# heng-hw/SpaCap3D

Hardware: AMD Instinct MI355X
Metric: scenes/sec (40k pts, 256 proposals) fwd+bwd (higher is better)
Workload: dtype f32; 1 GPU; cfg2: synthetic ScanRefer-shaped scans, 40000 pts x (xyz+1 ch), 256 proposals, 8 scenes/GPU; full training step (SpaCapNet fwd + loss + bwd + grad all-reduce + Adam); global_batch=8, parallelism=dp1, hip_graph=True, fps_prefetch_side_stream=True, prefetch_as_graph=True, reserved_cus_forward=8, geometry_prefetch=True, deferred_weight_gradients=True, params=9290918, allreduce_bytes=35572416

## Files before the change

### include/spacap_hip.h

```cpp
#ifndef SPACAP_HIP_H
#define SPACAP_HIP_H

#include <stddef.h>
#include <stdint.h>

#ifdef __cplusplus
extern "C" {
#endif

#define SPACAP_ABI_VERSION 5

#define SPACAP_OK 0
#define SPACAP_E_INVALID (-1)
#define SPACAP_E_LAUNCH (-2)
#define SPACAP_E_NO_DEVICE (-3)

typedef void *spacap_stream_t;

int spacap_abi_version(void);
const char *spacap_last_error(void);
int spacap_device_count(void);

int spacap_opt_n_threads(int work_size);

// ... 199 lines not shown
int spacap_sa_dgrad_l1in_f32(const float *dy, const float *zk, const float *coef, const float *Wk, const float *rel4,
                             const float *W1, int ldw, int has_feat, const float *st_p, int B, int N, int S, double *part,
                             float *part_l1, spacap_stream_t stream);
int spacap_sa_dgrad_wgrad_l1in_slabs(long R);
int spacap_sa_dgrad_wgrad_l1in_f32(const float *dy, const float *zk, const float *coef, const float *Wk, const float *rel4,
                                   const float *W1, int ldw, int has_feat, const float *st_p, int B, int N, int S, double *part,
                                   float *part_l1, float *partW, spacap_stream_t stream);
int spacap_sa_wgrad_f32(const float *dy, const uint8_t *arg, int S, const float *zk, const float *coef,
                        const float *zp, const float *st_p, long R, int CK, int CP, float *partW,
                        spacap_stream_t stream);
int spacap_sa_l1_bwd_f32(float *dy1, const float *z1, const float *coef, const float *feat, const float *xyz,
                         const float *new_xyz, const int32_t *idx, const float *W1, int ldw, float rdiv, int B,
                         int Np, int N, int S, int C1, float *partW, float *drel, int write_dz,
                         spacap_stream_t stream);
size_t spacap_sa_rows_scatter_workspace_bytes(int B, int Np, long E);
int spacap_sa_rows_scatter_f32(const float *dz, const int32_t *idx, int B, int Np, long E, int C, float *out,
                               void *workspace, spacap_stream_t stream);
int spacap_sa_rows_index_f32(const int32_t *idx, int B, int Np, long E, void *workspace, spacap_stream_t stream);
int spacap_sa_rows_gather_f32(const float *dz, int B, int Np, long E, int C, const void *workspace, float *out,
                              spacap_stream_t stream);
int spacap_sa_drel_sums_f32(const float *drel, int B, int Np, int N, int S, const void *workspace, float *dxyz, float *dnew,
                            spacap_stream_t stream);
int spacap_sa_dw1_assemble_f32(const float *pw1, int n1, const float *pf, int nf, int C1, int Cf, float *dW1, spacap_stream_t stream);

int spacap_linear_wgrad_slabs(long R, int CK, int CP);
int spacap_linear_wgrad_f32(const float *g, const float *x, long R, int CK, int CP, int with_bias, float *part,
                            spacap_stream_t stream);
int spacap_linear_wgrad_nslab_f32(const float *g, const float *x, long R, int CK, int CP, int with_bias, int nslab, float *part,
                                  spacap_stream_t stream);
int spacap_linear_wgrad_slabs_batched(long R, int CK, int CP);
int spacap_linear_wgrad_batched_f32(const float *const *g, const float *const *x, const long *R, const int *CK,
                                    const int *CP, const int *with_bias, const int *nslabs, float *const *part, int njobs,
                                    spacap_stream_t stream);

int spacap_relu_dropout_fwd_f32(const float *x, long n, float p, uint64_t seed, const uint64_t *seed_dev,
                                float *out, spacap_stream_t stream);
int spacap_relu_dropout_bwd_f32(const float *g, const float *y, long n, float p, float *dx, spacap_stream_t stream);
int spacap_dropout_add_fwd_f32(const float *res, const float *y, long n, float p, uint64_t seed,
                               const uint64_t *seed_dev, float *out, spacap_stream_t stream);
int spacap_dropout_add_bwd_f32(const float *g, long n, float p, uint64_t seed, const uint64_t *seed_dev,
                               float *out, spacap_stream_t stream);

int spacap_scene_aug_doubles(void);
int spacap_scene_sample_augment_f32(const float *const *scene_feat, const int32_t *const *scene_ins,
                                    const uint8_t *const *scene_isobj, const float *const *scene_color,
                                    const int32_t *choices, const double *aug, int B, int P, int C, int augment,
// ... 295 lines not shown
```

### spacap3d_amd/_native.py

```python
import ctypes
import os

import torch

_HERE = os.path.dirname(os.path.abspath(__file__))
LIB_PATH = os.path.join(_HERE, "lib", "libspacap_hip.so")
ABI_VERSION = 5

_i = ctypes.c_int
_l = ctypes.c_long
_f = ctypes.c_float
_p = ctypes.c_void_p
_u64 = ctypes.c_uint64

SIGNATURES = {
    "spacap_abi_version": (_i, []),
    "spacap_last_error": (ctypes.c_char_p, []),
    "spacap_device_count": (_i, []),
    "spacap_opt_n_threads": (_i, [_i]),
    "spacap_fps_workspace_bytes": (ctypes.c_size_t, [_i, _i]),
    "spacap_fps_f32": (_i, [_p, _i, _i, _i, _p, _p, _p]),
    "spacap_gather_points_f32": (_i, [_p, _p, _i, _i, _i, _i, _p, _p]),
    "spacap_gather_points_grad_f32": (_i, [_p, _p, _i, _i, _i, _i, _p, _p]),
    "spacap_ball_query_f32": (_i, [_p, _p, _i, _i, _i, _f, _i, _p, _p]),
# ... 112 lines not shown
    "spacap_rel_wide_tail_supported": (_i, [_i]),
    "spacap_rel_wide_tail_nparts": (_i, [_l]),
    "spacap_rel_wide_tail_bwd_f32": (_i, [_p, _p, _p, _l, _i, _i, _p, _p, _p]),
    "spacap_rel_wide_l1_supported": (_i, [_i, _i, _i]),
    "spacap_rel_wide_transpose_f32": (_i, [_p, _p, _i, _i, _i, _i, _p]),
    "spacap_rel_wide_l1_fwd_f32": (_i, [_p, _p, _p, _i, _i, _i, _i, _p, _p]),
    "spacap_rel_wide_l1_bwd_f32": (_i, [_p, _p, _p, _p, _i, _i, _i, _i, _p, _p, _p, _p]),
    "spacap_sa_l3bwd_part_floats": (_l, [_i, _i]),
    "spacap_sa_l3bwd_dw_f32": (_i, [_p, _i, _p, _p, _i, _i, _p, _p, _p]),
    "spacap_sa_wgrad_pool_supported": (_i, [_i, _i, _i]),
    "spacap_sa_wgrad_pool_parts": (_i, [_l, _i, _i, _i]),
    "spacap_sa_wgrad_pool_f32": (_i, [_p, _p, _i, _p, _p, _p, _l, _i, _i, _p, _p]),
    "spacap_sa_bwd_finalize_f32": (_i, [_p, _i, _l, _p, _p, _p, _p, _p]),
    "spacap_sa_dgrad_f32": (_i, [_p, _p, _i, _p, _p, _p, _p, _p, _l, _i, _i, _p, _p, _p]),
    "spacap_sa_dgrad_l1_f32": (_i, [_p] * 10 + [_f] + [_i] * 6 + [_p, _p, _p]),
    "spacap_sa_wgrad_f32": (_i, [_p, _p, _i, _p, _p, _p, _p, _l, _i, _i, _p, _p]),
    "spacap_sa_l1_bwd_f32": (_i, [_p, _p, _p, _p, _p, _p, _p, _p, _i, _f, _i, _i, _i, _i, _i, _p, _p, _i, _p]),
    "spacap_sa_rows_scatter_workspace_bytes": (ctypes.c_size_t, [_i, _i, _l]),
    "spacap_sa_rows_scatter_f32": (_i, [_p, _p, _i, _i, _l, _i, _p, _p, _p]),
    "spacap_sa_rows_index_f32": (_i, [_p, _i, _i, _l, _p, _p]),
    "spacap_sa_rows_gather_f32": (_i, [_p, _i, _i, _l, _i, _p, _p, _p]),
    "spacap_sa_drel_sums_f32": (_i, [_p, _i, _i, _i, _i, _p, _p, _p, _p]),
    "spacap_sa_dw1_assemble_f32": (_i, [_p, _i, _p, _i, _i, _i, _p, _p]),
    "spacap_relu_dropout_fwd_f32": (_i, [_p, _l, _f, _u64, _p, _p, _p]),
    "spacap_relu_dropout_bwd_f32": (_i, [_p, _p, _l, _f, _p, _p]),
    "spacap_dropout_add_fwd_f32": (_i, [_p, _p, _l, _f, _u64, _p, _p, _p]),
    "spacap_dropout_add_bwd_f32": (_i, [_p, _l, _f, _u64, _p, _p, _p]),
    "spacap_scene_aug_doubles": (_i, []),
    "spacap_scene_sample_augment_f32": (_i, [_p, _p, _p, _p, _p, _p, _i, _i, _i, _i, _p, _p, _p, _p, _p]),
    "spacap_scene_sample_augment_map_f32": (_i, [_p, _p, _p, _p, _p, _p, _i, _i, _i, _i, _i, _p, _p, _p, _p, _p, _p]),
    "spacap_scene_gather_rows_f32": (_i, [_p, _p, _i, _i, _i, _p, _i, _i, _p]),
    "spacap_l2norm_rows_fwd_f32": (_i, [_p, _l, _i, _p, _p, _p]),
    "spacap_l2norm_rows_bwd_f32": (_i, [_p, _p, _p, _l, _i, _p, _p]),
    "spacap_cap_loss_fwd_f32": (_i, [_p, _p, _p, _i, _i, _i, _i, _p, _p, _p, _p]),
    "spacap_cap_loss_bwd_f32": (_i, [_p, _p, _p, _p, _p, _i, _i, _i, _i, _p, _p]),
    "spacap_scene_votes_workspace_bytes": (ctypes.c_size_t, [_i, _i]),
    "spacap_scene_votes_f32": (_i, [_p, _p, _p, _i, _i, _i, _i, _p, _p, _p, _p]),
    "spacap_det_npart": (_i, []),
    "spacap_det_losses_fwd_f32": (_i, [_p] * 16 + [_i] * 8 + [_f] * 4 + [_p] * 9 + [_p]),
    "spacap_det_losses_bwd_f32": (_i, [_p] * 5 + [_i] * 6 + [_p] * 3 + [_p]),
    "spacap_rel_loss_nparts": (_l, [_i, _i]),
    "spacap_rel_loss_fwd_f32": (_i, [_p] * 7 + [_i] * 3 + [_p] * 3 + [_p]),
    "spacap_rel_loss_bwd_f32": (_i, [_p] * 3 + [_i] * 2 + [_p, _p]),
    "spacap_sum_slabs_f32": (_i, [_p, _i, _l, _p, _p]),
    "spacap_sum_slabs_batched_f32": (_i, [_p, _p, _p, _p, _i, _p]),
    "spacap_adam_flat_f32": (_i, [_p, _p, _p, _p, _l, _f, _f, _f, _f, _f, _p, _f, _p, _p]),
# ... 61 lines not shown
            "`python -c 'import __graft_entry__ as g; g.build()'` (or `make -C spacap3d_amd/csrc`). "
            "spacap3d_amd has no CPU or PyTorch fallback for its native operators.")
    lib = ctypes.CDLL(LIB_PATH)
    for name, (res, args) in SIGNATURES.items():
        fn = getattr(lib, name)
        fn.restype = res
        fn.argtypes = args
    got = lib.spacap_abi_version()
    if got != ABI_VERSION:
        raise ImportError(f"libspacap_hip.so ABI {got} != expected {ABI_VERSION}: rebuild the extension")
    return lib


lib = _load()


def check(rc: int, what: str) -> None:
    if rc != 0:
        msg = lib.spacap_last_error().decode("utf-8", "replace")
        raise RuntimeError(f"{what} failed (code {rc}): {msg}")


_DEFERRED = None


class deferred_slab_sums:

    def __enter__(self):
        global _DEFERRED
        self._prev = _DEFERRED
        self.items = []
        self.jobs = []
        self.conv_jobs = []
        _DEFERRED = self
        return self

    def __exit__(self, *exc):
        global _DEFERRED
        _DEFERRED = self._prev
        if exc[0] is None:
            self.flush()
        return False

    def has_job_for(self, part):
        ptr = part.data_ptr()
        return any(j[3].data_ptr() == ptr for j in self.jobs) or any(j[3].data_ptr() == ptr for j in self.conv_jobs)

    def outputs(self):
        return [o for _, o in self.items]

    def flush(self):
        self.run_jobs()
        self.run_sums()

    def run_jobs(self):
        import torch
        jobs, self.jobs = self.jobs, []
        if jobs:
            by_dev = {}
            for j in jobs:
                by_dev.setdefault(j[0].device, []).append(j)
            for dev, group in by_dev.items():
                k = len(group)
                arr = lambda ct, vals: (ct * k)(*vals)
                with torch.cuda.device(dev):
                    check(lib.spacap_linear_wgrad_batched_f32(
                        arr(ctypes.c_void_p, [j[0].data_ptr() for j in group]), arr(ctypes.c_void_p, [j[1].data_ptr() for j in group]),
                        arr(ctypes.c_long, [j[0].shape[0] for j in group]), arr(ctypes.c_int, [j[0].shape[1] for j in group]),
                        arr(ctypes.c_int, [j[1].shape[1] for j in group]), arr(ctypes.c_int, [int(j[2]) for j in group]),
                        arr(ctypes.c_int, [j[3].shape[0] for j in group]),
                        arr(ctypes.c_void_p, [j[3].data_ptr() for j in group]), k, torch.cuda.current_stream(dev).cuda_stream),
                        "spacap_linear_wgrad_batched_f32")
        cjobs, self.conv_jobs = self.conv_jobs, []
        if cjobs:
            by_dev = {}
            for j in cjobs:
# ... 61 lines not shown
            return out.view(part.shape[1:])
        return part[0]
    can_defer = deferrable and _DEFERRED is not None and part.is_cuda and part.data_ptr() % 16 == 0 and n % 4 == 0 \
        and part.dtype == torch.float32 and part.is_contiguous()
    if not can_defer and _DEFERRED is not None and part.is_cuda and _DEFERRED.has_job_for(part):
        _DEFERRED.run_jobs()
    if not part.is_cuda or n % 4 or part.dtype != torch.float32 or not part.is_contiguous():
        return part.sum(0)
    if can_defer:
        if out is None:
            with torch.cuda.device(part.device):
                out = torch.empty(part.shape[1:], dtype=torch.float32, device=part.device)
        else:
            out = out.view(part.shape[1:])
        _DEFERRED.items.append((part, out))
        return out
    with torch.cuda.device(part.device):
        out = torch.empty(part.shape[1:], dtype=torch.float32, device=part.device) if out is None else out.view(part.shape[1:])
        check(lib.spacap_sum_slabs_f32(part.data_ptr(), part.shape[0], n, out.data_ptr(),
                                       torch.cuda.current_stream(part.device).cuda_stream), "spacap_sum_slabs_f32")
    return out


def linear_wgrad_partials(g2, x2, with_bias, deferrable=False):
    import torch
    R, CK = g2.shape
    CP = x2.shape[1]
    nslab = int(lib.spacap_linear_wgrad_slabs(R, CK, CP))
    if nslab == 0:
        return None
    with torch.cuda.device(g2.device):
        if deferrable and _DEFERRED is not None:
            nb = int(lib.spacap_linear_wgrad_slabs_batched(R, CK, CP))
            part = torch.empty(nb, CK * CP + (CK if with_bias else 0), dtype=torch.float32, device=g2.device)
            _DEFERRED.jobs.append((g2, x2, bool(with_bias), part))
            return part
        part = torch.empty(nslab, CK * CP + (CK if with_bias else 0), dtype=torch.float32, device=g2.device)
        check(lib.spacap_linear_wgrad_f32(g2.data_ptr(), x2.data_ptr(), R, CK, CP, 1 if with_bias else 0, part.data_ptr(),
                                          torch.cuda.current_stream(g2.device).cuda_stream), "spacap_linear_wgrad_f32")
    return part


def conv1x1_wgrad_partials(g, x, B, CO, CI, N, deferrable=False, with_bias=False):
    import torch
    with torch.cuda.device(g.device):
        if deferrable and _DEFERRED is not None:
            nb = int(lib.spacap_conv1x1_wgrad_slabs_batched(B, CO, CI, N))
            part = torch.empty(nb, CO * CI + (((CO + 3) // 4) * 4 if with_bias else 0), dtype=torch.float32, device=g.device)
            _DEFERRED.conv_jobs.append((g, x, (B, CO, CI, N), part, bool(with_bias)))
            return part
        nslab = int(lib.spacap_conv1x1_wgrad_slabs(B, CO, CI, N))
        part = torch.empty(nslab, CO * CI, dtype=torch.float32, device=g.device)
        check(lib.spacap_conv1x1_wgrad_f32(g.data_ptr(), x.data_ptr(), B, CO, CI, N, part.data_ptr(),
                                           torch.cuda.current_stream(g.device).cuda_stream), "spacap_conv1x1_wgrad_f32")
    return part

# ... 20 lines not shown
```

### spacap3d_amd/csrc/sa_bwd.hip

```cpp
#include "sa_common.hpp"

namespace {

__global__ __launch_bounds__(1024) void sa_bwd_finalize_kernel(const double *__restrict__ part, int nparts, int C,
                                                              double M, const float *__restrict__ stats,
                                                              float *__restrict__ coef, float *__restrict__ dgamma,
                                                              float *__restrict__ dbeta) {
  __shared__ double s[64][16];
  const int tid = threadIdx.x, col = tid & 15, slab = tid >> 4;
  const int k = col >> 3, c = blockIdx.x * 8 + (col & 7);
  double a = 0.0;
  if (c < C) {
#pragma unroll 16
    for (int p = slab; p < nparts; p += 64) a += part[((size_t)p * 2 + k) * C + c];
  }
  s[slab][col] = a;
  __syncthreads();
  if (tid < 8 && c < C) {
    double s1 = 0.0, s2 = 0.0;
    for (int i = 0; i < 64; ++i) s1 += s[i][tid], s2 += s[i][tid + 8];
    const float mean = stats[c * 4], istd = stats[c * 4 + 1], g = stats[c * 4 + 2];
    const float a1 = (float)(s1 / M), b1 = (float)(s2 / M);
    const float k1 = g * b1 * istd;
    coef[c * 4 + 0] = g;
// ... 467 lines not shown
        py = dz[0] * wy[0] + dz[1] * wy[1] + dz[2] * wy[2] + dz[3] * wy[3];
        pz = dz[0] * wz[0] + dz[1] * wz[1] + dz[2] * wz[2] + dz[3] * wz[3];
      }
    }
    if (drel) {
#pragma unroll
      for (int o = 1; o < C4; o <<= 1) px += __shfl_xor(px, o), py += __shfl_xor(py, o), pz += __shfl_xor(pz, o);
      if (c4 == 0 && r < R) drel[r * 3] = px / rdiv, drel[r * 3 + 1] = py / rdiv, drel[r * 3 + 2] = pz / rdiv;
    }
  }
  st4(&s_red[0][rs][c4 * 4], ax);
  st4(&s_red[1][rs][c4 * 4], ay);
  st4(&s_red[2][rs][c4 * 4], az);
  st4(&s_red[3][rs][c4 * 4], af);
  __syncthreads();
  for (int e = tid; e < 4 * C1; e += 256) {
    const int c = e / 4, k = e % 4;
    float a = 0.f;
    for (int i = 0; i < RP; ++i) a += s_red[k][i][c];
    partW[((size_t)blockIdx.x * C1 + c) * 4 + k] = a;
  }
}

__global__ __launch_bounds__(256) void sa_dw1_assemble_kernel(const float *__restrict__ pw1, int n1, const float *__restrict__ pf, int nf,
                                                              int C1, int Cf, float *__restrict__ out) {
  __shared__ float s_g[4][64];
  const int c = threadIdx.x & 63, grp = threadIdx.x >> 6;
  const long e = (long)blockIdx.x * 64 + c, ne = (long)C1 * (3 + Cf);
  float a = 0.f;
  if (e < ne) {
    const int ch = (int)(e / (3 + Cf)), j = (int)(e % (3 + Cf));
    const float *src = j < 3 ? pw1 + (size_t)ch * 4 + j : pf + (size_t)ch * Cf + (j - 3);
    const size_t stride = j < 3 ? (size_t)C1 * 4 : (size_t)C1 * Cf;
    const int ns = j < 3 ? n1 : nf, per = (ns + 3) / 4, s0 = grp * per, s1 = min(ns, s0 + per);
    int k = s0;
    for (; k + 32 <= s1; k += 32) {
      float t[32];
#pragma unroll
      for (int u = 0; u < 32; ++u) t[u] = src[(size_t)(k + u) * stride];
#pragma unroll
      for (int u = 0; u < 32; ++u) a += t[u];
    }
#pragma unroll 8
    for (; k < s1; ++k) a += src[(size_t)k * stride];
  }
  s_g[grp][c] = a;
  __syncthreads();
  if (grp == 0 && e < ne) out[e] = (s_g[0][c] + s_g[1][c]) + (s_g[2][c] + s_g[3][c]);
}

}

namespace {
int wgrad_resident(int CK, int CP, bool pooled) {
#define WR(CKB, CPV, PV)                                                        \
  {                                                                             \
    static const int res = resident_blocks(sa_wgrad_kernel<CKB, CPV, PV>, 0);   \
    return res;                                                                 \
  }
  if (pooled && CK % 128 == 0 && CP == 64) WR(128, 64, true)
  if (pooled && CK % 128 == 0 && CP == 128) WR(128, 128, true)
  if (!pooled && CK == 64 && CP == 64) WR(64, 64, false)
  if (!pooled && CK == 128 && CP == 128) WR(128, 128, false)
#undef WR
  return 512;
}
}
extern "C" int spacap_sa_wgrad_slabs(long R, int CK, int CP, int pooled) {
  const int gy = CK >= 128 ? CK / 128 : 1;
  long n = bwd_resident(wgrad_resident(CK, CP, pooled != 0)) / gy, cap = (16L << 20) / ((long)CK * CP), tiles = (R + TW - 1) / TW;
  if (n > cap) n = cap;
// ... 161 lines not shown
  const char *what = "spacap_sa_dgrad_l1in_f32";
  SPACAP_REQUIRE(dy && zk && coef && Wk && rel4 && W1 && st_p && part && part_l1 && ldw >= (has_feat ? 4 : 3), "%s: bad arguments", what);
  const long R = (long)B * N * S;
  L1Args L{nullptr, nullptr, nullptr, nullptr, 1.f, 1, N, S, part_l1, rel4, L1In{W1, ldw, has_feat}, nullptr};
  launch_dgrad_l1<false>(dy, zk, coef, Wk, nullptr, st_p, R, part, L, spacap::as_stream(stream));
  SPACAP_CHECK_LAUNCH(what);
  return SPACAP_OK;
}

extern "C" int spacap_sa_dgrad_wgrad_l1in_slabs(long R) { return R >= 1 ? dgrad_l1_grid<true>(R) : 0; }
extern "C" int spacap_sa_dgrad_wgrad_l1in_f32(const float *dy, const float *zk, const float *coef, const float *Wk, const float *rel4,
                                              const float *W1, int ldw, int has_feat, const float *st_p, int B, int N, int S,
                                              double *part, float *part_l1, float *partW, spacap_stream_t stream) {
  const char *what = "spacap_sa_dgrad_wgrad_l1in_f32";
  SPACAP_REQUIRE(dy && zk && coef && Wk && rel4 && W1 && st_p && part && part_l1 && partW && ldw >= (has_feat ? 4 : 3), "%s: bad arguments", what);
  const long R = (long)B * N * S;
  L1Args L{nullptr, nullptr, nullptr, nullptr, 1.f, 1, N, S, part_l1, rel4, L1In{W1, ldw, has_feat}, partW};
  launch_dgrad_l1<true>(dy, zk, coef, Wk, nullptr, st_p, R, part, L, spacap::as_stream(stream));
  SPACAP_CHECK_LAUNCH(what);
  return SPACAP_OK;
}

namespace {
__global__ __launch_bounds__(256) void sa_l1_dw_kernel(const float *__restrict__ part_l1, int nparts, const float *__restrict__ coef,
                                                       int C1, int ldw, float *__restrict__ dW1) {
  __shared__ double s_lane[12][17];
  __shared__ double s_sum[12];
  const int c = blockIdx.x, tid = threadIdx.x, sidx = tid >> 4, l = tid & 15;
  const int n = C1 * 8 + 4;
  if (sidx < 12) {
    const int e = sidx < 8 ? c * 8 + sidx : C1 * 8 + (sidx - 8);
    double a0 = 0.0, a1 = 0.0, a2 = 0.0, a3 = 0.0;
    int p = l;
    for (; p + 48 < nparts; p += 64) {
      a0 += (double)part_l1[(size_t)p * n + e];
      a1 += (double)part_l1[(size_t)(p + 16) * n + e];
      a2 += (double)part_l1[(size_t)(p + 32) * n + e];
      a3 += (double)part_l1[(size_t)(p + 48) * n + e];
    }
    for (; p < nparts; p += 16) a0 += (double)part_l1[(size_t)p * n + e];
    s_lane[sidx][l] = (a0 + a1) + (a2 + a3);
  }
  __syncthreads();
  if (tid < 12) {
    double a = 0.0;
    for (int i = 0; i < 16; ++i) a += s_lane[tid][i];
    s_sum[tid] = a;
  }
  __syncthreads();
  if (tid < ldw) {
    const double g = coef[c * 4 + 0], k0 = coef[c * 4 + 1], k1 = coef[c * 4 + 2];
    dW1[c * ldw + tid] = (float)(g * s_sum[tid] + k0 * s_sum[8 + tid] - k1 * s_sum[4 + tid]);
  }
}
}
extern "C" int spacap_sa_l1_dw_f32(const float *part_l1, int nparts, const float *coef, int C1, int ldw, float *dW1,
                                   spacap_stream_t stream) {
  const char *what = "spacap_sa_l1_dw_f32";
  SPACAP_REQUIRE(part_l1 && coef && dW1 && nparts >= 1 && C1 >= 1 && C1 <= 512 && ldw >= 1 && ldw <= 4, "%s: bad arguments", what);
  hipLaunchKernelGGL(sa_l1_dw_kernel, dim3(C1), dim3(256), 0, spacap::as_stream(stream), part_l1, nparts, coef, C1, ldw, dW1);
  SPACAP_CHECK_LAUNCH(what);
  return SPACAP_OK;
}

extern "C" int spacap_sa_wgrad_f32(const float *dy, const uint8_t *arg, int S, const float *zk, const float *coef,
                                   const float *zp, const float *st_p, long R, int CK, int CP, float *partW,
                                   spacap_stream_t stream) {
  const char *what = "spacap_sa_wgrad_f32";
  SPACAP_REQUIRE(dy && zk && coef && zp && st_p && partW && R >= 1, "%s: bad arguments", what);
  SPACAP_REQUIRE(!arg || (S >= 1 && R % S == 0), "%s: bad S", what);
  hipStream_t s = spacap::as_stream(stream);
  const int nslab = spacap_sa_wgrad_slabs(R, CK, CP, arg ? 1 : 0);
#define WG(CKB, CPV, PV) \
  hipLaunchKernelGGL((sa_wgrad_kernel<CKB, CPV, PV>), dim3(nslab, CK / CKB), dim3(256), 0, s, dy, arg, S, zk, coef, CK, zp, st_p, R, partW)
  if (arg && CK % 128 == 0 && CP == 64) WG(128, 64, true);
  else if (arg && CK % 128 == 0 && CP == 128) WG(128, 128, true);
  else if (!arg && CK == 64 && CP == 64) WG(64, 64, false);
  else if (!arg && CK == 128 && CP == 128) WG(128, 128, false);
  else SPACAP_REQUIRE(false, "%s: (CK=%d, CP=%d, pooled=%d) unsupported", what, CK, CP, arg ? 1 : 0);
#undef WG
  SPACAP_CHECK_LAUNCH(what);
  return SPACAP_OK;
}
// ... 28 lines not shown
```

### spacap3d_amd/csrc/sa_l3bwd.inc

```

__global__ __launch_bounds__(256) void sa_l3_sum_kernel(const float *__restrict__ partW, int nparts, long n, double *__restrict__ sums) {
  __shared__ double s_l[16][65];
  const int q = threadIdx.x & 15, l = threadIdx.x >> 4;
  const long e0 = (long)blockIdx.x * 64 + q * 4;
  double a[4] = {0.0, 0.0, 0.0, 0.0};
  if (e0 < n) {
    const float *pp = partW + e0;
    int p = l;
    for (; p + 7 * 16 < nparts; p += 8 * 16) {
      f32x4 t[8];
#pragma unroll
      for (int u = 0; u < 8; ++u) t[u] = ld4(pp + (size_t)(p + 16 * u) * n);
#pragma unroll
      for (int u = 0; u < 8; ++u)
#pragma unroll
        for (int k = 0; k < 4; ++k) a[k] += (double)t[u][k];
    }
    for (; p < nparts; p += 16) {
      const f32x4 t = ld4(pp + (size_t)p * n);
#pragma unroll
      for (int k = 0; k < 4; ++k) a[k] += (double)t[k];
    }
  }
#pragma unroll
  for (int k = 0; k < 4; ++k) s_l[l][q * 4 + k] = a[k];
  __syncthreads();
  if (threadIdx.x < 64 && (long)blockIdx.x * 64 + threadIdx.x < n) {
    double v = 0.0;
    for (int i = 0; i < 16; ++i) v += s_l[i][threadIdx.x];
    sums[(long)blockIdx.x * 64 + threadIdx.x] = v;
  }
}

__global__ __launch_bounds__(1024) void sa_l3_dw_kernel(const double *__restrict__ sums, const float *__restrict__ coef3,
                                                        const float *__restrict__ W3, int C3, int C2, float *__restrict__ dW3) {
  __shared__ double s_p[1024];
  const int c = blockIdx.x, k = threadIdx.x % C2, sl = threadIdx.x / C2, nsl = 1024 / C2;
  const double *gram = sums + (size_t)C3 * C2, *cs = gram + (size_t)C2 * C2;
  double acc = 0.0;
  for (int j0 = sl * 8; j0 < C2; j0 += nsl * 8) {
    double gv[8];
    float wv[8];
#pragma unroll
    for (int u = 0; u < 8; ++u) {
      const int j = j0 + u < C2 ? j0 + u : C2 - 1;
      gv[u] = gram[(size_t)j * C2 + k];
      wv[u] = W3[(size_t)c * C2 + j];
    }
#pragma unroll
    for (int u = 0; u < 8; ++u)
      if (j0 + u < C2) acc += (double)wv[u] * gv[u];
  }
  s_p[threadIdx.x] = acc;
  __syncthreads();
  if (threadIdx.x < C2) {
    double v = 0.0;
    for (int i = 0; i < nsl; ++i) v += s_p[i * C2 + threadIdx.x];
    const double k0 = coef3[c * 4 + 1], k1 = coef3[c * 4 + 2];
    dW3[(size_t)c * C2 + threadIdx.x] = (float)(sums[(size_t)c * C2 + threadIdx.x] + k0 * cs[threadIdx.x] - k1 * v);
  }
}

struct WPArgs {
  const float *dym;
  const uint8_t *arg;
  const float *coef3;
  const float *z2;
  const float *st2;
  long R;
  float *partW;
};

template <int W, int C2, int C3, int TMT, int S>
__device__ __forceinline__ void wp_tile(const float *sa, const float *sv, const int *sr, f32x4 (&accG)[C2 / 32 + 1],
                                        float (&sacc)[C3 / (C2 / 16)][C2 / 64], int lane) {
  constexpr int NCL = C2 / 16, CH = C2 / 64, CPL = C2 / 64, NI = C3 / NCL, ND = NCL / 2 + 1, NDW = W < NCL / 2 ? ND : ND - 1;
  constexpr int LDA = C2 + 20, KS = TMT / 4, NG = TMT / S, IPK = NG * NI / KS;
  static_assert((NG * NI) % KS == 0 && NI % 4 == 0 && (IPK % 4 == 0 || 4 % IPK == 0), "sparse items per k step");
  using i32x4 = int __attribute__((ext_vector_type(4)));
  const int l15 = lane & 15, lg = lane >> 4;
  const float *pb = sa + lg * LDA + 4 * l15;
  const float *psp = sa + CPL * lane;
  const f32x4 *qv = reinterpret_cast<const f32x4 *>(sv) + W * (NI / 4);
// ... 167 lines not shown
```

### spacap3d_amd/engine.py

```python
import os

import torch

from . import synthetic as S
from .detector import geometry_pyramid, sampling_pyramid
from .distributed import FlatGradBucket, broadcast_parameters, used_parameters
from .loss_helper import get_scene_cap_loss, start_detection_losses


_STREAMS = {}


def _role_stream(device, role):
    device = torch.device(device)
    key = (device.type, device.index if device.index is not None else torch.cuda.current_device())
    if key not in _STREAMS:
        dev = torch.device("cuda", key[1])
        _STREAMS[key] = {r: torch.cuda.Stream(device=dev) for r in ("side", "capture", "comm", "wgrad", "relation")}
    return _STREAMS[key][role]


class Trainer:
    def __init__(self, model: torch.nn.Module, mean_size_arr, lr: float = 1e-3, weight_decay: float = 1e-5,
                 use_relation: bool = True, split_optimizer: bool = False,
# ... 106 lines not shown
        kw = dict(num_heading_bin=S.NUM_HEADING_BIN, num_size_cluster=S.NUM_SIZE_CLUSTER, mean_size_arr=self.mean_size_arr)
        need = ("vote_label", "center_label")
        early = (lambda d: start_detection_losses(d, **kw)) if all(k in data_dict for k in need) else None
        d = self.model(dict(data_dict), after_proposal=early)
        det_vec = d.get("_det_vec")
        d = get_scene_cap_loss(d, use_relation=self.use_relation, **kw)
        if self._overlap_armed or self._flush_mid:
            marks = [t for t in (det_vec, d.get("aggregated_vote_features"), d.get("aggregated_vote_xyz"))
                     if torch.is_tensor(t) and t.requires_grad]
            for t in marks:
                t.register_hook(self._boundary_hook if self._overlap_armed else self._mid_flush_hook)
        return d

    def _mid_flush_hook(self, grad):
        if self._flush_mid and not self._mid_done:
            self._mid_done = 1
            from . import _native
            dq = _native._DEFERRED
            if dq is not None and grad.is_cuda:
                dev = grad.device
                ws = _role_stream(dev, "wgrad")
                cur = torch.cuda.current_stream(dev)
                ws.wait_stream(cur)
                for j in dq.jobs + dq.conv_jobs:
                    for t in (j[0], j[1], j[3]):
                        t.record_stream(ws)
                for part, out in dq.items:
                    part.record_stream(ws)
                    out.record_stream(ws)
                with torch.cuda.stream(ws):
                    dq.flush()
                self._mid_stream = ws
        return None

    def _setup(self, data_dict):
        bufs = [(b, b.detach().clone()) for b in self.model.buffers()]
        d = self.loss(data_dict)
        used = used_parameters(self.model, d["loss"])
        with torch.no_grad():
            for b, saved in bufs:
                b.copy_(saved)
        used = self._group_qkv(used)
        self._adopt_bn_counters()
        self.bucket = FlatGradBucket(used, views=False)
        kw = dict(lr=self.lr, weight_decay=self.weight_decay, eps=self.adam_eps)
        if used[0].is_cuda:
            from .optim import FlatAdam
            self.optimizer = FlatAdam(self.bucket, **kw)
            self._attach_packed_qkv()
            self._register_grad_slots()
        else:
            self.optimizer = torch.optim.Adam(used, **kw)
# ... 504 lines not shown
```

### spacap3d_amd/sa_mlp.py

```python
import torch
from torch.autograd import Function

from .layout import ChannelMajorOf, point_major_of
from ._native import check, lib, sum_slabs


RECOMPUTE_Z1 = True
L1_MOMENTS = True
POOL_WGRAD = True
POOL_WGRAD_MIN_ROWS = 131072
FUSE_L2_WGRAD = True


def _ptr(t):
    return t.data_ptr() if t is not None else None


_SELFTESTED = set()


def _selftest(dev):
    key = (dev.type, dev.index)
    if key in _SELFTESTED:
        return
    _SELFTESTED.add(key)
    with torch.cuda.device(dev), torch.no_grad():
# ... 147 lines not shown
        nparts = int(lib.spacap_sa_nparts())
        with torch.cuda.device(dev):
            part = torch.empty(nparts * 2 * max(C1, C2, C3), dtype=torch.float64, device=dev)
            coef = [torch.empty(c, 4, **f32) for c in (C1, C2, C3)]
            dg = [torch.empty(c, **f32) for c in (C1, C2, C3)]
            db = [torch.empty(c, **f32) for c in (C1, C2, C3)]

            def finalize(k, C, stats):
                check(lib.spacap_sa_bwd_finalize_f32(part.data_ptr(), C, R, stats.data_ptr(), coef[k].data_ptr(),
                                                     dg[k].data_ptr(), db[k].data_ptr(), st), "spacap_sa_bwd_finalize_f32")

            dym = torch.empty(G, C3, **f32)
            check(lib.spacap_sa_pool_bwd_f32(dout.data_ptr(), out.data_ptr(), arg.data_ptr(), z3.data_ptr(), _ptr(zmax), st3.data_ptr(), G, S, C3,
                                             dym.data_ptr(), part.data_ptr(), st), "spacap_sa_pool_bwd_f32")
            finalize(2, C3, st3)
            dy2 = torch.empty(R, C2, **f32)
            if POOL_WGRAD and R >= POOL_WGRAD_MIN_ROWS and lib.spacap_sa_wgrad_pool_supported(C2, C3, S):
                npw, nfl = int(lib.spacap_sa_wgrad_pool_parts(R, C2, C3, S)), int(lib.spacap_sa_l3bwd_part_floats(C2, C3))
                pw = torch.empty(npw, nfl, **f32)
                check(lib.spacap_sa_wgrad_pool_f32(dym.data_ptr(), arg.data_ptr(), S, coef[2].data_ptr(), z2.data_ptr(),
                                                   st2.data_ptr(), R, C3, C2, pw.data_ptr(), st), "spacap_sa_wgrad_pool_f32")
                sums = torch.empty(nfl, dtype=torch.float64, device=dev)
                dW3 = torch.empty(C3, C2, **f32)
                check(lib.spacap_sa_l3bwd_dw_f32(pw.data_ptr(), npw, coef[2].data_ptr(), W3.data_ptr(), C3, C2, sums.data_ptr(),
                                                 dW3.data_ptr(), st), "spacap_sa_l3bwd_dw_f32")
            else:
                pw = torch.empty(int(lib.spacap_sa_wgrad_slabs(R, C3, C2, 1)), C3, C2, **f32)
                check(lib.spacap_sa_wgrad_f32(dym.data_ptr(), arg.data_ptr(), S, z3.data_ptr(), coef[2].data_ptr(),
                                              z2.data_ptr(), st2.data_ptr(), R, C3, C2, pw.data_ptr(), st), "spacap_sa_wgrad_f32")
                dW3 = sum_slabs(pw, deferrable=True)
            check(lib.spacap_sa_dgrad_f32(dym.data_ptr(), arg.data_ptr(), S, z3.data_ptr(), coef[2].data_ptr(),
                                          W3.data_ptr(), z2.data_ptr(), st2.data_ptr(), R, C3, C2, dy2.data_ptr(),
                                          part.data_ptr(), st), "spacap_sa_dgrad_f32")
            finalize(1, C2, st2)
            has_feat = int(feat is not None)
            fuse_l1 = (not ctx.has_Y) and (not ctx.need_xyz) and C1 == 64 and C2 == 64
            fuse_w2 = fuse_l1 and ctx.recompute and FUSE_L2_WGRAD
            if fuse_w2:
                pw = torch.empty(int(lib.spacap_sa_dgrad_wgrad_l1in_slabs(R)), C2, C1, **f32)
            else:
                pw = torch.empty(int(lib.spacap_sa_wgrad_slabs(R, C2, C1, 0)), C2, C1, **f32)
                if ctx.recompute:
                    check(lib.spacap_sa_wgrad_l1in_f32(dy2.data_ptr(), z2.data_ptr(), coef[1].data_ptr(), z1.data_ptr(), W1.data_ptr(),
                                                       W1.shape[1], has_feat, st1.data_ptr(), R, pw.data_ptr(), st),
                          "spacap_sa_wgrad_l1in_f32")
                else:
                    check(lib.spacap_sa_wgrad_f32(dy2.data_ptr(), None, 0, z2.data_ptr(), coef[1].data_ptr(), z1.data_ptr(),
                                                  st1.data_ptr(), R, C2, C1, pw.data_ptr(), st), "spacap_sa_wgrad_f32")
                dW2 = sum_slabs(pw, deferrable=True)
            if fuse_l1:
                pl1 = torch.empty(nparts, C1 * 8 + 4, **f32)
                if fuse_w2:
                    check(lib.spacap_sa_dgrad_wgrad_l1in_f32(dy2.data_ptr(), z2.data_ptr(), coef[1].data_ptr(), W2.data_ptr(),
                                                             z1.data_ptr(), W1.data_ptr(), W1.shape[1], has_feat, st1.data_ptr(), B, N, S,
                                                             part.data_ptr(), pl1.data_ptr(), pw.data_ptr(), st),
                          "spacap_sa_dgrad_wgrad_l1in_f32")
                    dW2 = sum_slabs(pw, deferrable=True)
                elif ctx.recompute:
                    check(lib.spacap_sa_dgrad_l1in_f32(dy2.data_ptr(), z2.data_ptr(), coef[1].data_ptr(), W2.data_ptr(),
                                                       z1.data_ptr(), W1.data_ptr(), W1.shape[1], has_feat, st1.data_ptr(), B, N, S,
                                                       part.data_ptr(), pl1.data_ptr(), st), "spacap_sa_dgrad_l1in_f32")
                else:
                    check(lib.spacap_sa_dgrad_l1_f32(dy2.data_ptr(), z2.data_ptr(), coef[1].data_ptr(), W2.data_ptr(),
                                                     z1.data_ptr(), st1.data_ptr(), _ptr(feat), xyz.data_ptr(),
                                                     new_xyz.data_ptr(), idx.data_ptr(), ctx.rdiv, B, Np, N, S, C2, C1,
                                                     part.data_ptr(), pl1.data_ptr(), st), "spacap_sa_dgrad_l1_f32")
                del dy2
                finalize(0, C1, st1)
                dW1 = torch.empty(C1, W1.shape[1], **f32)
                check(lib.spacap_sa_l1_dw_f32(pl1.data_ptr(), nparts, coef[0].data_ptr(), C1, W1.shape[1], dW1.data_ptr(), st),
                      "spacap_sa_l1_dw_f32")
                return (None, None, None, None, None, dW1, dW2, dW3, dg[0], db[0], dg[1], db[1], dg[2], db[2], None, None, None)
            dy1 = torch.empty(R, C1, **f32)
            check(lib.spacap_sa_dgrad_f32(dy2.data_ptr(), None, 0, z2.data_ptr(), coef[1].data_ptr(), W2.data_ptr(),
                                          z1.data_ptr(), st1.data_ptr(), R, C2, C1, dy1.data_ptr(), part.data_ptr(), st),
                  "spacap_sa_dgrad_f32")
            del dy2
            finalize(0, C1, st1)
            pw1 = torch.empty(nparts, C1, 4, **f32)
            drel = torch.empty(R, 3, **f32) if ctx.need_xyz else None
            check(lib.spacap_sa_l1_bwd_f32(dy1.data_ptr(), z1.data_ptr(), coef[0].data_ptr(), _ptr(feat), xyz.data_ptr(),
                                           new_xyz.data_ptr(), idx.data_ptr(), W1.data_ptr(), W1.shape[1], ctx.rdiv, B, Np,
                                           N, S, C1, pw1.data_ptr(), _ptr(drel), int(ctx.has_Y), st),
                  "spacap_sa_l1_bwd_f32")
            dY = ws = None
            nbytes = int(lib.spacap_sa_rows_scatter_workspace_bytes(B, Np, N * S))
            ri = ctx.rows_index
            if ri is not None and not (ri.numel() == nbytes and ri.device == dev):
                ri = None
            if ctx.has_Y:
                dY = torch.empty(B, Np, C1, **f32)
                if ri is not None:
                    check(lib.spacap_sa_rows_gather_f32(dy1.data_ptr(), B, Np, N * S, C1, ri.data_ptr(), dY.data_ptr(), st),
                          "spacap_sa_rows_gather_f32")
                else:
                    ws = torch.empty(nbytes, dtype=torch.uint8, device=dev)
                    check(lib.spacap_sa_rows_scatter_f32(dy1.data_ptr(), idx.data_ptr(), B, Np, N * S, C1, dY.data_ptr(),
                                                         ws.data_ptr(), st), "spacap_sa_rows_scatter_f32")
            dpm = None
            if ctx.has_Y:
                pm = ctx.pm
                Cf = W1.shape[1] - 3
                g2, x2 = dY.view(-1, C1), _rows2d(pm)
                if ctx.needs_input_grad[4]:
                    from .linear import dense_product
                    dpm = dense_product(g2, W1, False, col0=3).view_as(pm)
                nslab = int(lib.spacap_linear_wgrad_slabs(B * Np, C1, Cf))
                if nslab:
                    x2c = x2.contiguous()
                    pf = torch.empty(nslab, C1 * Cf, **f32)
                    check(lib.spacap_linear_wgrad_f32(g2.data_ptr(), x2c.data_ptr(), B * Np, C1, Cf, 0, pf.data_ptr(), st),
                          "spacap_linear_wgrad_f32")
                else:
                    nslab = int(lib.spacap_dense_wgrad_tall_slabs(B * Np, C1, Cf))
                    pf = torch.empty(nslab, C1 * Cf, **f32)
                    check(lib.spacap_dense_wgrad_tall_f32(g2.data_ptr(), C1, x2.data_ptr(), x2.stride(0), B * Np, C1, Cf, nslab,
                                                          pf.data_ptr(), st), "spacap_dense_wgrad_tall_f32")
                dW1 = torch.empty(C1, 3 + Cf, **f32)
                check(lib.spacap_sa_dw1_assemble_f32(pw1.data_ptr(), nparts, pf.data_ptr(), nslab, C1, Cf, dW1.data_ptr(), st),
                      "spacap_sa_dw1_assemble_f32")
            else:
                dW1 = sum_slabs(pw1)[:, :W1.shape[1]].contiguous()
            dxyz = dnew = None
            if drel is not None:
                want_x, want_n = ctx.needs_input_grad[0], ctx.needs_input_grad[1]
                if want_x and ri is None and ws is None:
                    ws = torch.empty(nbytes, dtype=torch.uint8, device=dev)
                    check(lib.spacap_sa_rows_index_f32(idx.data_ptr(), B, Np, N * S, ws.data_ptr(), st), "spacap_sa_rows_index_f32")
                index = ri if ri is not None else ws
                dxyz = torch.empty(B, Np, 3, **f32) if want_x else None
                dnew = torch.empty(B, N, 3, **f32) if want_n else None
                if want_x or want_n:
                    check(lib.spacap_sa_drel_sums_f32(drel.data_ptr(), B, Np, N, S, _ptr(index) if want_x else None, _ptr(dxyz), _ptr(dnew),
                                                      st), "spacap_sa_drel_sums_f32")
        return (dxyz, dnew, None, None, dpm, dW1, dW2, dW3, dg[0], db[0], dg[1], db[1], dg[2], db[2], None, None, None)


def _uniform_rows(pm):
    return pm.stride(2) == 1 and pm.stride(0) == pm.shape[1] * pm.stride(1) and pm.data_ptr() % 4 == 0


def _rows2d(pm):
    B, Np, Cf = pm.shape
# ... 109 lines not shown
```

Baseline: 1196 scenes/s.

## Defer SA-layer weight-gradient finish kernels into batched launches on wgrad stream

The small per-layer SA weight-gradient finishing kernels (l3 partial sums, l3 dW, dW1 assembly, l1 dW) are now queued in the deferred weight-gradient context. They run as a few multi-job batched launches, using a block-to-job table, on the side wgrad stream instead of inline in the backward pass. The SA dW1 feature-wgrad slabs are also routed through the deferred linear-wgrad batch. This cuts launch count and moves tail work off the critical backward path. The cost is extra bookkeeping, tensor lifetime tracking via record_stream, and binary-search job dispatch inside the kernels.

```diff
diff --git a/include/spacap_hip.h b/include/spacap_hip.h
--- a/include/spacap_hip.h
+++ b/include/spacap_hip.h
@@ -245,6 +245,14 @@
 int spacap_sa_drel_sums_f32(const float *drel, int B, int Np, int N, int S, const void *workspace, float *dxyz, float *dnew,
                             spacap_stream_t stream);
 int spacap_sa_dw1_assemble_f32(const float *pw1, int n1, const float *pf, int nf, int C1, int Cf, float *dW1, spacap_stream_t stream);
+#define SPACAP_SA_FINISH_L3_SUM 0
+#define SPACAP_SA_FINISH_L3_DW 1
+#define SPACAP_SA_FINISH_DW1_ASSEMBLE 2
+#define SPACAP_SA_FINISH_L1_DW 3
+int spacap_sa_finish_job_max(void);
+int spacap_sa_finish_batched_f32(const int *kind, const void *const *a, const float *const *b, const float *const *c,
+                                 void *const *out, const int *n0, const int *n1, const int *d0, const int *d1, int njobs,
+                                 spacap_stream_t stream);
 
 int spacap_linear_wgrad_slabs(long R, int CK, int CP);
 int spacap_linear_wgrad_f32(const float *g, const float *x, long R, int CK, int CP, int with_bias, float *part,
diff --git a/spacap3d_amd/_native.py b/spacap3d_amd/_native.py
--- a/spacap3d_amd/_native.py
+++ b/spacap3d_amd/_native.py
@@ -158,6 +158,8 @@
     "spacap_sa_rows_gather_f32": (_i, [_p, _i, _i, _l, _i, _p, _p, _p]),
     "spacap_sa_drel_sums_f32": (_i, [_p, _i, _i, _i, _i, _p, _p, _p, _p]),
     "spacap_sa_dw1_assemble_f32": (_i, [_p, _i, _p, _i, _i, _i, _p, _p]),
+    "spacap_sa_finish_job_max": (_i, []),
+    "spacap_sa_finish_batched_f32": (_i, [_p] * 9 + [_i, _p]),
     "spacap_relu_dropout_fwd_f32": (_i, [_p, _l, _f, _u64, _p, _p, _p]),
     "spacap_relu_dropout_bwd_f32": (_i, [_p, _p, _l, _f, _p, _p]),
     "spacap_dropout_add_fwd_f32": (_i, [_p, _p, _l, _f, _u64, _p, _p, _p]),
@@ -265,6 +267,7 @@
 
 
 _DEFERRED = None
+SA_L3_SUM, SA_L3_DW, SA_DW1_ASSEMBLE, SA_L1_DW = 0, 1, 2, 3
 
 
 class deferred_slab_sums:
@@ -275,6 +278,7 @@
         self.items = []
         self.jobs = []
         self.conv_jobs = []
+        self.sa_jobs = []
         _DEFERRED = self
         return self
 
@@ -290,11 +294,46 @@
         return any(j[3].data_ptr() == ptr for j in self.jobs) or any(j[3].data_ptr() == ptr for j in self.conv_jobs)
 
     def outputs(self):
-        return [o for _, o in self.items]
+        return [o for _, o in self.items] + [j[1] for j in self.sa_jobs]
+
+    def tensors(self):
+        ts = [t for j in self.jobs + self.conv_jobs for t in (j[0], j[1], j[3])]
+        ts += [t for pair in self.items for t in pair]
+        ts += [t for j in self.sa_jobs for t in (j[1],) + tuple(j[2])]
+        return ts
 
     def flush(self):
         self.run_jobs()
+        self.run_sa_jobs()
         self.run_sums()
+
+    def sa_finish(self, kind, out, reads, ints):
+        self.sa_jobs.append((kind, out, tuple(reads), tuple(int(v) for v in ints)))
+        return out
+
+    def run_sa_jobs(self):
+        import torch
+        jobs, self.sa_jobs = self.sa_jobs, []
+        by_dev = {}
+        for j in jobs:
+            by_dev.setdefault(j[1].device, []).append(j)
+        for dev, group in by_dev.items():
+            rows = []
+            for kind, out, reads, ints in group:
+                if kind == SA_L3_DW:
+                    rows.append((SA_L3_SUM, reads[0].data_ptr(), None, None, reads[1].data_ptr(), ints[0], 0, ints[1], ints[2]))
+                    rows.append((SA_L3_DW, reads[1].data_ptr(), reads[2].data_ptr(), reads[3].data_ptr(), out.data_ptr(), 0, 0, ints[1], ints[2]))
+                elif kind == SA_DW1_ASSEMBLE:
+                    rows.append((kind, reads[0].data_ptr(), reads[1].data_ptr(), None, out.data_ptr(), ints[0], ints[1], ints[2], ints[3]))
+                else:
+                    rows.append((kind, reads[0].data_ptr(), reads[1].data_ptr(), None, out.data_ptr(), ints[0], 0, ints[1], ints[2]))
+            k = len(rows)
+            col = lambda ct, i: (ct * k)(*[r[i] for r in rows])
+            with torch.cuda.device(dev):
+                check(lib.spacap_sa_finish_batched_f32(
+                    col(ctypes.c_int, 0), col(ctypes.c_void_p, 1), col(ctypes.c_void_p, 2), col(ctypes.c_void_p, 3), col(ctypes.c_void_p, 4),
+                    col(ctypes.c_int, 5), col(ctypes.c_int, 6), col(ctypes.c_int, 7), col(ctypes.c_int, 8), k,
+                    torch.cuda.current_stream(dev).cuda_stream), "spacap_sa_finish_batched_f32")
 
     def run_jobs(self):
         import torch
@@ -402,7 +441,7 @@
     return out
 
 
-def linear_wgrad_partials(g2, x2, with_bias, deferrable=False):
+def linear_wgrad_partials(g2, x2, with_bias, deferrable=False, single_launch_slabs=False):
     import torch
     R, CK = g2.shape
     CP = x2.shape[1]
@@ -411,7 +450,7 @@
         return None
     with torch.cuda.device(g2.device):
         if deferrable and _DEFERRED is not None:
-            nb = int(lib.spacap_linear_wgrad_slabs_batched(R, CK, CP))
+            nb = nslab if single_launch_slabs else int(lib.spacap_linear_wgrad_slabs_batched(R, CK, CP))
             part = torch.empty(nb, CK * CP + (CK if with_bias else 0), dtype=torch.float32, device=g2.device)
             _DEFERRED.jobs.append((g2, x2, bool(with_bias), part))
             return part
diff --git a/spacap3d_amd/csrc/sa_bwd.hip b/spacap3d_amd/csrc/sa_bwd.hip
--- a/spacap3d_amd/csrc/sa_bwd.hip
+++ b/spacap3d_amd/csrc/sa_bwd.hip
@@ -513,11 +513,11 @@
   }
 }
 
-__global__ __launch_bounds__(256) void sa_dw1_assemble_kernel(const float *__restrict__ pw1, int n1, const float *__restrict__ pf, int nf,
-                                                              int C1, int Cf, float *__restrict__ out) {
+__device__ __forceinline__ void sa_dw1_assemble_body(const float *__restrict__ pw1, int n1, const float *__restrict__ pf, int nf, int C1,
+                                                     int Cf, float *__restrict__ out, int blk) {
   __shared__ float s_g[4][64];
   const int c = threadIdx.x & 63, grp = threadIdx.x >> 6;
-  const long e = (long)blockIdx.x * 64 + c, ne = (long)C1 * (3 + Cf);
+  const long e = (long)blk * 64 + c, ne = (long)C1 * (3 + Cf);
   float a = 0.f;
   if (e < ne) {
     const int ch = (int)(e / (3 + Cf)), j = (int)(e % (3 + Cf));
@@ -538,6 +538,10 @@
   s_g[grp][c] = a;
   __syncthreads();
   if (grp == 0 && e < ne) out[e] = (s_g[0][c] + s_g[1][c]) + (s_g[2][c] + s_g[3][c]);
+}
+__global__ __launch_bounds__(256) void sa_dw1_assemble_kernel(const float *__restrict__ pw1, int n1, const float *__restrict__ pf, int nf,
+                                                              int C1, int Cf, float *__restrict__ out) {
+  sa_dw1_assemble_body(pw1, n1, pf, nf, C1, Cf, out, (int)blockIdx.x);
 }
 
 }
@@ -745,11 +749,11 @@
 }
 
 namespace {
-__global__ __launch_bounds__(256) void sa_l1_dw_kernel(const float *__restrict__ part_l1, int nparts, const float *__restrict__ coef,
-                                                       int C1, int ldw, float *__restrict__ dW1) {
+__device__ __forceinline__ void sa_l1_dw_body(const float *__restrict__ part_l1, int nparts, const float *__restrict__ coef, int C1,
+                                              int ldw, float *__restrict__ dW1, int blk) {
   __shared__ double s_lane[12][17];
   __shared__ double s_sum[12];
-  const int c = blockIdx.x, tid = threadIdx.x, sidx = tid >> 4, l = tid & 15;
+  const int c = blk, tid = threadIdx.x, sidx = tid >> 4, l = tid & 15;
   const int n = C1 * 8 + 4;
   if (sidx < 12) {
     const int e = sidx < 8 ? c * 8 + sidx : C1 * 8 + (sidx - 8);
@@ -776,12 +780,102 @@
     dW1[c * ldw + tid] = (float)(g * s_sum[tid] + k0 * s_sum[8 + tid] - k1 * s_sum[4 + tid]);
   }
 }
-}
+__global__ __launch_bounds__(256) void sa_l1_dw_kernel(const float *__restrict__ part_l1, int nparts, const float *__restrict__ coef,
+                                                       int C1, int ldw, float *__restrict__ dW1) {
+  sa_l1_dw_body(part_l1, nparts, coef, C1, ldw, dW1, (int)blockIdx.x);
+}
+
+constexpr int SA_FIN_JOB_MAX = 8;
+struct SaFinJob {
+  const void *a;
+  const float *b;
+  const float *c;
+  void *out;
+  int kind, block0;
+  int n0, n1;
+  int d0, d1;
+};
+struct SaFinTable {
+  int njobs, pad;
+  SaFinJob job[SA_FIN_JOB_MAX];
+};
+__device__ __forceinline__ SaFinJob fin_job_of_block(const SaFinTable &T) {
+  int lo = 0, hi = T.njobs - 1;
+  while (lo < hi) {
+    const int mid = (lo + hi + 1) >> 1;
+    if (T.job[mid].block0 <= (int)blockIdx.x) lo = mid; else hi = mid - 1;
+  }
+  return T.job[lo];
+}
+__global__ __launch_bounds__(256) void sa_finish_batched_kernel(const SaFinTable T) {
+  const SaFinJob J = fin_job_of_block(T);
+  const int blk = (int)blockIdx.x - J.block0;
+  if (J.kind == SPACAP_SA_FINISH_L3_SUM)
+    sa_l3_sum_body(static_cast<const float *>(J.a), J.n0, (long)J.d0 * J.d1 + (long)J.d1 * J.d1 + J.d1, static_cast<double *>(J.out), blk);
+  else if (J.kind == SPACAP_SA_FINISH_DW1_ASSEMBLE)
+    sa_dw1_assemble_body(static_cast<const float *>(J.a), J.n0, J.b, J.n1, J.d0, J.d1, static_cast<float *>(J.out), blk);
+  else
+    sa_l1_dw_body(static_cast<const float *>(J.a), J.n0, J.b, J.d0, J.d1, static_cast<float *>(J.out), blk);
+}
+__global__ __launch_bounds__(1024) void sa_l3_dw_batched_kernel(const SaFinTable T) {
+  const SaFinJob J = fin_job_of_block(T);
+  sa_l3_dw_body(static_cast<const double *>(J.a), J.b, J.c, J.d0, J.d1, static_cast<float *>(J.out), (int)blockIdx.x - J.block0);
+}
+}
+
 extern "C" int spacap_sa_l1_dw_f32(const float *part_l1, int nparts, const float *coef, int C1, int ldw, float *dW1,
                                    spacap_stream_t stream) {
   const char *what = "spacap_sa_l1_dw_f32";
   SPACAP_REQUIRE(part_l1 && coef && dW1 && nparts >= 1 && C1 >= 1 && C1 <= 512 && ldw >= 1 && ldw <= 4, "%s: bad arguments", what);
   hipLaunchKernelGGL(sa_l1_dw_kernel, dim3(C1), dim3(256), 0, spacap::as_stream(stream), part_l1, nparts, coef, C1, ldw, dW1);
+  SPACAP_CHECK_LAUNCH(what);
+  return SPACAP_OK;
+}
+
+extern "C" int spacap_sa_finish_job_max(void) { return SA_FIN_JOB_MAX; }
+
+extern "C" int spacap_sa_finish_batched_f32(const int *kind, const void *const *a, const float *const *b, const float *const *c,
+                                            void *const *out, const int *n0, const int *n1, const int *d0, const int *d1, int njobs,
+                                            spacap_stream_t stream) {
+  const char *what = "spacap_sa_finish_batched_f32";
+  SPACAP_REQUIRE(njobs >= 0 && (njobs == 0 || (kind && a && b && c && out && n0 && n1 && d0 && d1)), "%s: bad arguments", what);
+  for (int i = 0; i < njobs; ++i) {
+    SPACAP_REQUIRE(a[i] && out[i], "%s: job %d: null pointer", what, i);
+    if (kind[i] == SPACAP_SA_FINISH_L3_SUM)
+      SPACAP_REQUIRE(n0[i] >= 1 && d0[i] >= 1 && d1[i] >= 4 && d1[i] % 4 == 0 && spacap::aligned16(a[i]),
+                     "%s: job %d: l3 sums: bad arguments or partW not 16-byte aligned", what, i);
+    else if (kind[i] == SPACAP_SA_FINISH_L3_DW)
+      SPACAP_REQUIRE(b[i] && c[i] && d0[i] >= 1 && d1[i] >= 4 && d1[i] % 4 == 0 && d1[i] <= 1024 && 1024 % d1[i] == 0,
+                     "%s: job %d: l3 dW (C3=%d, C2=%d) unsupported or null pointer", what, i, d0[i], d1[i]);
+    else if (kind[i] == SPACAP_SA_FINISH_DW1_ASSEMBLE)
+      SPACAP_REQUIRE(b[i] && n0[i] >= 1 && n1[i] >= 1 && d0[i] >= 1 && d1[i] >= 1, "%s: job %d: dW1 assemble: bad arguments", what, i);
+    else if (kind[i] == SPACAP_SA_FINISH_L1_DW)
+      SPACAP_REQUIRE(b[i] && n0[i] >= 1 && d0[i] >= 1 && d0[i] <= 512 && d1[i] >= 1 && d1[i] <= 4, "%s: job %d: l1 dW: bad arguments", what, i);
+    else
+      SPACAP_REQUIRE(false, "%s: job %d: kind %d unknown", what, i, kind[i]);
+  }
+  hipStream_t s = spacap::as_stream(stream);
+  for (int wide = 0; wide < 2; ++wide) {
+    int i = 0;
+    while (i < njobs) {
+      SaFinTable T;
+      T.njobs = 0, T.pad = 0;
+      long blocks = 0;
+      for (; i < njobs && T.njobs < SA_FIN_JOB_MAX; ++i) {
+        if ((kind[i] == SPACAP_SA_FINISH_L3_DW) != (wide != 0)) continue;
+        SaFinJob &J = T.job[T.njobs++];
+        J.a = a[i], J.b = b[i], J.c = c[i], J.out = out[i], J.kind = kind[i], J.block0 = (int)blocks;
+        J.n0 = n0[i], J.n1 = n1[i], J.d0 = d0[i], J.d1 = d1[i];
+        if (kind[i] == SPACAP_SA_FINISH_L3_SUM) blocks += nblocks(spacap_sa_l3bwd_part_floats(d1[i], d0[i]), 64);
+        else if (kind[i] == SPACAP_SA_FINISH_DW1_ASSEMBLE) blocks += nblocks((long)d0[i] * (3 + d1[i]), 64);
+        else blocks += d0[i];
+        SPACAP_REQUIRE(blocks < 2147483647L, "%s: too many blocks", what);
+      }
+      if (T.njobs == 0) continue;
+      if (wide) hipLaunchKernelGGL(sa_l3_dw_batched_kernel, dim3((unsigned)blocks), dim3(1024), 0, s, T);
+      else hipLaunchKernelGGL(sa_finish_batched_kernel, dim3((unsigned)blocks), dim3(256), 0, s, T);
+    }
+  }
   SPACAP_CHECK_LAUNCH(what);
   return SPACAP_OK;
 }
diff --git a/spacap3d_amd/csrc/sa_l3bwd.inc b/spacap3d_amd/csrc/sa_l3bwd.inc
--- a/spacap3d_amd/csrc/sa_l3bwd.inc
+++ b/spacap3d_amd/csrc/sa_l3bwd.inc
@@ -1,8 +1,8 @@
 
-__global__ __launch_bounds__(256) void sa_l3_sum_kernel(const float *__restrict__ partW, int nparts, long n, double *__restrict__ sums) {
+__device__ __forceinline__ void sa_l3_sum_body(const float *__restrict__ partW, int nparts, long n, double *__restrict__ sums, int blk) {
   __shared__ double s_l[16][65];
   const int q = threadIdx.x & 15, l = threadIdx.x >> 4;
-  const long e0 = (long)blockIdx.x * 64 + q * 4;
+  const long e0 = (long)blk * 64 + q * 4;
   double a[4] = {0.0, 0.0, 0.0, 0.0};
   if (e0 < n) {
     const float *pp = partW + e0;
@@ -25,17 +25,20 @@
 #pragma unroll
   for (int k = 0; k < 4; ++k) s_l[l][q * 4 + k] = a[k];
   __syncthreads();
-  if (threadIdx.x < 64 && (long)blockIdx.x * 64 + threadIdx.x < n) {
+  if (threadIdx.x < 64 && (long)blk * 64 + threadIdx.x < n) {
     double v = 0.0;
     for (int i = 0; i < 16; ++i) v += s_l[i][threadIdx.x];
-    sums[(long)blockIdx.x * 64 + threadIdx.x] = v;
-  }
-}
-
-__global__ __launch_bounds__(1024) void sa_l3_dw_kernel(const double *__restrict__ sums, const float *__restrict__ coef3,
-                                                        const float *__restrict__ W3, int C3, int C2, float *__restrict__ dW3) {
+    sums[(long)blk * 64 + threadIdx.x] = v;
+  }
+}
+__global__ __launch_bounds__(256) void sa_l3_sum_kernel(const float *__restrict__ partW, int nparts, long n, double *__restrict__ sums) {
+  sa_l3_sum_body(partW, nparts, n, sums, (int)blockIdx.x);
+}
+
+__device__ __forceinline__ void sa_l3_dw_body(const double *__restrict__ sums, const float *__restrict__ coef3,
+                                              const float *__restrict__ W3, int C3, int C2, float *__restrict__ dW3, int blk) {
   __shared__ double s_p[1024];
-  const int c = blockIdx.x, k = threadIdx.x % C2, sl = threadIdx.x / C2, nsl = 1024 / C2;
+  const int c = blk, k = threadIdx.x % C2, sl = threadIdx.x / C2, nsl = 1024 / C2;
   const double *gram = sums + (size_t)C3 * C2, *cs = gram + (size_t)C2 * C2;
   double acc = 0.0;
   for (int j0 = sl * 8; j0 < C2; j0 += nsl * 8) {
@@ -59,6 +62,10 @@
     const double k0 = coef3[c * 4 + 1], k1 = coef3[c * 4 + 2];
     dW3[(size_t)c * C2 + threadIdx.x] = (float)(sums[(size_t)c * C2 + threadIdx.x] + k0 * cs[threadIdx.x] - k1 * v);
   }
+}
+__global__ __launch_bounds__(1024) void sa_l3_dw_kernel(const double *__restrict__ sums, const float *__restrict__ coef3,
+                                                        const float *__restrict__ W3, int C3, int C2, float *__restrict__ dW3) {
+  sa_l3_dw_body(sums, coef3, W3, C3, C2, dW3, (int)blockIdx.x);
 }
 
 struct WPArgs {
diff --git a/spacap3d_amd/engine.py b/spacap3d_amd/engine.py
--- a/spacap3d_amd/engine.py
+++ b/spacap3d_amd/engine.py
@@ -152,12 +152,8 @@
                 ws = _role_stream(dev, "wgrad")
                 cur = torch.cuda.current_stream(dev)
                 ws.wait_stream(cur)
-                for j in dq.jobs + dq.conv_jobs:
-                    for t in (j[0], j[1], j[3]):
-                        t.record_stream(ws)
-                for part, out in dq.items:
-                    part.record_stream(ws)
-                    out.record_stream(ws)
+                for t in dq.tensors():
+                    t.record_stream(ws)
                 with torch.cuda.stream(ws):
                     dq.flush()
                 self._mid_stream = ws
diff --git a/spacap3d_amd/sa_mlp.py b/spacap3d_amd/sa_mlp.py
--- a/spacap3d_amd/sa_mlp.py
+++ b/spacap3d_amd/sa_mlp.py
@@ -2,6 +2,7 @@
 from torch.autograd import Function
 
 from .layout import ChannelMajorOf, point_major_of
+from . import _native
 from ._native import check, lib, sum_slabs
 
 
@@ -195,8 +196,12 @@
                                                    st2.data_ptr(), R, C3, C2, pw.data_ptr(), st), "spacap_sa_wgrad_pool_f32")
                 sums = torch.empty(nfl, dtype=torch.float64, device=dev)
                 dW3 = torch.empty(C3, C2, **f32)
-                check(lib.spacap_sa_l3bwd_dw_f32(pw.data_ptr(), npw, coef[2].data_ptr(), W3.data_ptr(), C3, C2, sums.data_ptr(),
-                                                 dW3.data_ptr(), st), "spacap_sa_l3bwd_dw_f32")
+                dq = _native._DEFERRED
+                if dq is not None:
+                    dq.sa_finish(_native.SA_L3_DW, dW3, (pw, sums, coef[2], W3), (npw, C3, C2))
+                else:
+                    check(lib.spacap_sa_l3bwd_dw_f32(pw.data_ptr(), npw, coef[2].data_ptr(), W3.data_ptr(), C3, C2, sums.data_ptr(),
+                                                     dW3.data_ptr(), st), "spacap_sa_l3bwd_dw_f32")
             else:
                 pw = torch.empty(int(lib.spacap_sa_wgrad_slabs(R, C3, C2, 1)), C3, C2, **f32)
                 check(lib.spacap_sa_wgrad_f32(dym.data_ptr(), arg.data_ptr(), S, z3.data_ptr(), coef[2].data_ptr(),
@@ -241,8 +246,12 @@
                 del dy2
                 finalize(0, C1, st1)
                 dW1 = torch.empty(C1, W1.shape[1], **f32)
-                check(lib.spacap_sa_l1_dw_f32(pl1.data_ptr(), nparts, coef[0].data_ptr(), C1, W1.shape[1], dW1.data_ptr(), st),
-                      "spacap_sa_l1_dw_f32")
+                dq = _native._DEFERRED
+                if dq is not None:
+                    dq.sa_finish(_native.SA_L1_DW, dW1, (pl1, coef[0]), (nparts, C1, W1.shape[1]))
+                else:
+                    check(lib.spacap_sa_l1_dw_f32(pl1.data_ptr(), nparts, coef[0].data_ptr(), C1, W1.shape[1], dW1.data_ptr(), st),
+                          "spacap_sa_l1_dw_f32")
                 return (None, None, None, None, None, dW1, dW2, dW3, dg[0], db[0], dg[1], db[1], dg[2], db[2], None, None, None)
             dy1 = torch.empty(R, C1, **f32)
             check(lib.spacap_sa_dgrad_f32(dy2.data_ptr(), None, 0, z2.data_ptr(), coef[1].data_ptr(), W2.data_ptr(),
@@ -278,20 +287,22 @@
                 if ctx.needs_input_grad[4]:
                     from .linear import dense_product
                     dpm = dense_product(g2, W1, False, col0=3).view_as(pm)
+                dq = _native._DEFERRED
                 nslab = int(lib.spacap_linear_wgrad_slabs(B * Np, C1, Cf))
                 if nslab:
-                    x2c = x2.contiguous()
-                    pf = torch.empty(nslab, C1 * Cf, **f32)
-                    check(lib.spacap_linear_wgrad_f32(g2.data_ptr(), x2c.data_ptr(), B * Np, C1, Cf, 0, pf.data_ptr(), st),
-                          "spacap_linear_wgrad_f32")
-                else:
+                    pf = _native.linear_wgrad_partials(g2, x2.contiguous(), False, deferrable=True, single_launch_slabs=True)
+                else:
+                    dq = None
                     nslab = int(lib.spacap_dense_wgrad_tall_slabs(B * Np, C1, Cf))
                     pf = torch.empty(nslab, C1 * Cf, **f32)
                     check(lib.spacap_dense_wgrad_tall_f32(g2.data_ptr(), C1, x2.data_ptr(), x2.stride(0), B * Np, C1, Cf, nslab,
                                                           pf.data_ptr(), st), "spacap_dense_wgrad_tall_f32")
                 dW1 = torch.empty(C1, 3 + Cf, **f32)
-                check(lib.spacap_sa_dw1_assemble_f32(pw1.data_ptr(), nparts, pf.data_ptr(), nslab, C1, Cf, dW1.data_ptr(), st),
-                      "spacap_sa_dw1_assemble_f32")
+                if dq is not None:
+                    dq.sa_finish(_native.SA_DW1_ASSEMBLE, dW1, (pw1, pf), (nparts, nslab, C1, Cf))
+                else:
+                    check(lib.spacap_sa_dw1_assemble_f32(pw1.data_ptr(), nparts, pf.data_ptr(), nslab, C1, Cf, dW1.data_ptr(), st),
+                          "spacap_sa_dw1_assemble_f32")
             else:
                 dW1 = sum_slabs(pw1)[:, :W1.shape[1]].contiguous()
             dxyz = dnew = None
```

After: 1204 scenes/s, median of 6. Within noise of the previous version (+0.6%).
